# chrischoy/DeepGlobalRegistration

Hardware: AMD Instinct MI355X
Metric: pair registrations/sec (FCGF x2 + 1-NN + 6-D inlier net + gate + weighted Procrustes + SE(3) refinement) (higher is better)
Workload: dtype f32 results via 2 x f16 split operands (3 f16 MFMA products per MAC, f32 accumulate); k = 1 convs, kNN re-evaluation and registration in exact f32, SVD in f64

## Files before the change

deepglobalregistration_amd/_lib.py:

```python
import ctypes as C
import os
import threading

import torch

_HERE = os.path.dirname(os.path.abspath(__file__))
LIB_PATH = os.environ.get('DGR_HIP_LIB') or os.path.join(_HERE, 'lib', 'libdgr_hip.so')

DGR_OK, DGR_EINVAL, DGR_EHIP, DGR_ENOMEM, DGR_ESVD, DGR_EINTERNAL = 0, -1, -2, -3, -4, -5
STATUS_OK, STATUS_LOW_CONFIDENCE, STATUS_SVD_FAILED, STATUS_SAFEGUARD = 0, 1, 2, 3
STATUS_FLAG_ICP_SKIPPED, STATUS_MASK = 0x100, 0xff

c_i32p, c_i64p, c_f32p, c_f64p = (C.POINTER(C.c_int32), C.POINTER(C.c_int64),
                                  C.POINTER(C.c_float), C.POINTER(C.c_double))
vp = C.c_void_p


class WeightDesc(C.Structure):
    _fields_ = [('name', C.c_char_p), ('data', vp), ('numel', C.c_int64)]


class Params(C.Structure):
    _fields_ = [('clip_weight_thresh', C.c_float), ('voxel_size', C.c_float),
                ('inlier_feature_type', C.c_int), ('max_iter', C.c_int),
# ... 12 lines not shown
    'dgr_ctx_create': (C.c_int, [C.c_int, C.POINTER(vp)]),
    'dgr_ctx_destroy': (None, [vp]),
    'dgr_ctx_workspace_bytes': (C.c_int64, [vp]),
    'dgr_ctx_create_partition_stream': (C.c_int, [vp, C.c_int, C.c_int, C.POINTER(vp)]),
    'dgr_voxelize': (C.c_int, [vp, vp, C.c_int, C.c_int64, C.c_double, C.c_int32, vp, vp, vp, c_i64p, vp]),
    'dgr_net_create': (C.c_int, [vp, C.c_int, C.c_int, C.c_int, C.c_int, C.c_int,
                                 C.POINTER(WeightDesc), C.c_int, C.POINTER(vp)]),
    'dgr_net_create_device': (C.c_int, [vp, C.c_int, C.c_int, C.c_int, C.c_int, C.c_int,
                                        C.POINTER(WeightDesc), C.c_int, C.POINTER(vp)]),
    'dgr_net_destroy': (None, [vp]),
    'dgr_net_param_bytes': (C.c_int64, [vp]),
    'dgr_net_share': (C.c_int, [vp, vp, C.POINTER(vp)]),
    'dgr_net_sharers': (C.c_int, [vp]),
    'dgr_resunet_forward': (C.c_int, [vp, vp, vp, vp, C.c_int64, vp, vp]),
    'dgr_net_get_intermediate': (C.c_int, [vp, vp, C.c_char_p, vp, C.c_int64, c_i64p, c_i64p]),
    'dgr_net_layer_stats': (C.c_int, [vp, vp, C.c_int, c_i64p]),
    'dgr_net_num_layers': (C.c_int, [vp]),
    'dgr_net_rerun_layer': (C.c_int, [vp, vp, C.c_int, C.c_int, c_f32p, c_f32p]),
    'dgr_maps_create': (C.c_int, [vp, vp, C.c_int64, C.c_int, C.c_int, C.POINTER(vp), vp]),
    'dgr_maps_destroy': (None, [vp]),
    'dgr_maps_get_coords': (C.c_int, [vp, C.c_int, vp, C.c_int64, c_i64p]),
    'dgr_maps_get_kernel_map': (C.c_int, [vp, C.c_int, C.c_int, vp, C.c_int64, vp, vp, C.c_int64,
                                          c_i64p, c_i64p]),
    'dgr_knn1_l2': (C.c_int, [vp, vp, C.c_int64, vp, C.c_int64, C.c_int, C.c_int, vp, vp, vp]),
    'dgr_knn1_l2_batch': (C.c_int, [vp, vp, c_i64p, vp, c_i64p, C.c_int, C.c_int, C.c_int, vp, vp, vp]),
    'dgr_knn_l2': (C.c_int, [vp, vp, C.c_int64, vp, C.c_int64, C.c_int, C.c_int, C.c_int, vp, vp, vp]),
    'dgr_knn_l2_batch': (C.c_int, [vp, vp, c_i64p, vp, c_i64p, C.c_int, C.c_int, C.c_int, C.c_int, vp, vp,
                                   vp]),
    'dgr_inlier_inputs': (C.c_int, [vp, vp, vp, C.c_int64, vp, vp, C.c_int64, vp, C.c_int, vp, vp, vp]),
    'dgr_sigmoid_clip_sum': (C.c_int, [vp, vp, C.c_int64, C.c_float, vp, c_f64p, vp]),
    'dgr_gather_rows3': (C.c_int, [vp, vp, vp, C.c_int64, vp, vp]),
    'dgr_weighted_procrustes': (C.c_int, [vp, vp, vp, vp, C.c_int64, C.c_float, c_f32p, c_f32p, vp]),
    'dgr_se3_refine': (C.c_int, [vp, vp, vp, vp, C.c_int64, C.c_float, C.c_int, C.c_int, C.c_double,
                                 c_f32p, c_f32p, c_i32p, c_f32p, c_i32p, vp]),
    'dgr_register_batch': (C.c_int, [vp, vp, vp, vp, vp, c_i64p, vp, vp, c_i64p, C.c_int,
                                     C.POINTER(Params), vp, vp, c_f32p, c_i32p, c_f32p, vp]),
    'dgr_register_pairs': (C.c_int, [vp, vp, vp, vp, vp, c_i64p, C.c_int, C.c_int, c_i32p, C.c_int,
                                     C.POINTER(Params), vp, vp, c_f32p, c_i32p, c_f32p, vp]),
    'dgr_register_batch_f64': (C.c_int, [vp, c_f64p, C.c_int64, c_i64p]),
    'dgr_register_batch_output': (C.c_int, [vp, C.c_int, vp, C.c_int64, c_i64p, vp]),
    'dgr_ctx_set_profiling': (C.c_int, [vp, C.c_int]),
    'dgr_icp_point_to_point': (C.c_int, [vp, vp, C.c_int64, vp, C.c_int64, C.c_double, c_f64p, C.c_int, C.c_double,
                                          C.c_double, c_f64p, c_f64p, vp]),
    'dgr_ransac_correspondence': (C.c_int, [vp, vp, vp, C.c_int64, C.c_double, C.c_int64, C.c_uint32, c_f64p, c_f64p, vp]),
    'dgr_ctx_stage_times': (C.c_int, [vp, c_f32p]),
    'dgr_ctx_stage_times_v2': (C.c_int, [vp, c_f32p, C.c_int, C.POINTER(C.c_int)]),
# ... 109 lines not shown
```

deepglobalregistration_amd/csrc/coordmap.hip:

```cpp
#include <algorithm>

#include "dgr_internal.h"
#include "hash.h"

constexpr int SCAN_THREADS = 256;
constexpr int SCAN_ITEMS = 8;
constexpr int SCAN_BLOCK = SCAN_THREADS * SCAN_ITEMS;

__device__ __forceinline__ int block_exclusive_scan_256(int v, int *lds , int *total) {
  const int lane = threadIdx.x & 63, wave = threadIdx.x >> 6;
  int x = v;
#pragma unroll
  for (int d = 1; d < 64; d <<= 1) {
    int y = __shfl_up(x, d, 64);
    if (lane >= d) x += y;
  }
  if (lane == 63) lds[wave] = x;
  __syncthreads();
  int base = 0, tot = 0;
#pragma unroll
  for (int w = 0; w < SCAN_THREADS / 64; ++w) {
    int s = lds[w];
    if (w < wave) base += s;
    tot += s;
// ... 288 lines not shown
}

__global__ void half_keys_kernel(const int32_t *__restrict__ coords7, const int32_t *n_dev,
                                 int32_t *__restrict__ keys4) {
  int64_t r = (int64_t)blockIdx.x * blockDim.x + threadIdx.x;
  if (r >= *n_dev) return;
#pragma unroll
  for (int d = 0; d < 4; ++d) keys4[r * 4 + d] = coords7[r * 7 + d];
}

__global__ void bucket_count_kernel(const int32_t *__restrict__ keys4, const int32_t *n_dev,
                                    const int32_t *__restrict__ table, uint32_t mask,
                                    const int32_t *__restrict__ bkeys, int32_t *__restrict__ row_bucket,
                                    int32_t *counts) {
  int64_t r = (int64_t)blockIdx.x * blockDim.x + threadIdx.x;
  if (r >= *n_dev) return;
  int32_t q[4] = {keys4[r * 4], keys4[r * 4 + 1], keys4[r * 4 + 2], keys4[r * 4 + 3]};
  const int b = dgr_lookup<4>(table, mask, bkeys, q);
  row_bucket[r] = b;
  atomicAdd(&counts[b], 1);
}

__global__ void bucket_members_kernel(const int32_t *__restrict__ row_bucket, const int32_t *n_dev,
                                      const int32_t *__restrict__ start, int32_t *cursor, int32_t *__restrict__ members) {
  int64_t r = (int64_t)blockIdx.x * blockDim.x + threadIdx.x;
  if (r >= *n_dev) return;
  const int b = row_bucket[r];
  members[start[b] + atomicAdd(&cursor[b], 1)] = (int32_t)r;
}

__global__ void bucket_fill_kernel(const int32_t *__restrict__ row_bucket, const int32_t *n_dev,
                                   const int32_t *__restrict__ start, int32_t *cursor,
                                   const int32_t *__restrict__ members,
                                   const int32_t *__restrict__ coords7, int4 *__restrict__ second,
                                   int32_t *__restrict__ coords_new, int32_t *__restrict__ canon, int32_t *__restrict__ inv) {
  int64_t r = (int64_t)blockIdx.x * blockDim.x + threadIdx.x;
  if (r >= *n_dev) return;
  const int b = row_bucket[r];
  const int32_t *c = coords7 + r * 7;
  int p;
  if (members) {
    int rank = 0;
    for (int e = start[b], end = start[b + 1]; e < end; ++e) rank += members[e] < (int32_t)r;
    p = start[b] + rank;
  } else {
    p = start[b] + atomicAdd(&cursor[b], 1);
  }
  if (coords_new) {
#pragma unroll
    for (int d = 0; d < 7; ++d) coords_new[(int64_t)p * 7 + d] = c[d];
    canon[p] = (int32_t)r;
    inv[r] = p;
    second[p] = make_int4(c[4], c[5], c[6], p);
  } else {
    second[p] = make_int4(c[4], c[5], c[6], (int32_t)r);
  }
}

struct RenumberJobs {
  const int32_t *inv[4];
  int32_t *table[4];
  uint32_t cap[4];
};
__global__ void renumber_table_kernel(RenumberJobs j) {
  const int l = blockIdx.y;
  const uint32_t s = blockIdx.x * blockDim.x + threadIdx.x;
  if (s >= j.cap[l]) return;
  const int v = j.table[l][s];
  if (v >= 0) j.table[l][s] = j.inv[l][v];
}
// ... 52 lines not shown
  }
  DGR_LAUNCH_CHECK();
  {
    const int32_t *ins[4];
    int32_t *outs[4], *tots[4];
    int64_t ns[4];
    for (int l = 0; l < levels; ++l) { ins[l] = counts[l]; outs[l] = hb[l].start; tots[l] = nullptr; ns[l] = cm[l].n_cap + 1; }
    DGR_CHECK(dgr_exclusive_scan_multi(arena, levels, ins, outs, ns, tots, stream));
  }
  RenumberJobs rj = {};
  int nrj = 0;
  int64_t max_cap = 0;
  for (int l = 0; l < levels; ++l) {
    const int64_t n = cm[l].n_cap;
    int32_t *coords_new = nullptr, *canon = nullptr, *inv = nullptr;
    if (l >= renumber_from) {
      DGR_ALLOC(coords_new, arena, int32_t, n * 7);
      DGR_ALLOC(canon, arena, int32_t, n);
      DGR_ALLOC(inv, arena, int32_t, n);
      rj.inv[nrj] = inv; rj.table[nrj] = cm[l].table; rj.cap[nrj] = cm[l].table_mask + 1;
      max_cap = std::max<int64_t>(max_cap, rj.cap[nrj]);
      ++nrj;
    }
    const int32_t *members = nullptr;
    if (coords_new) {
      bucket_members_kernel<<<grid_for(n), 256, 0, stream>>>(row_bucket[l], cm[l].n_dev, hb[l].start, cursor[l], rank[l]);
      members = rank[l];
    }
    bucket_fill_kernel<<<grid_for(n), 256, 0, stream>>>(row_bucket[l], cm[l].n_dev, hb[l].start, cursor[l], members,
                                                        cm[l].coords, hb[l].second, coords_new, canon, inv);
    if (coords_new) { cm[l].coords = coords_new; cm[l].canon = canon; }
    hb[l].built = true;
  }
  if (nrj) renumber_table_kernel<<<dim3((unsigned)grid_for(max_cap), nrj), 256, 0, stream>>>(rj);
  DGR_LAUNCH_CHECK();
  return DGR_OK;
}

int dgr_build_coord_maps(DgrArena &arena, const int32_t *coords, int64_t N, DgrMapSet *ms,
                         hipStream_t stream) {
  if (ms->nc == 4) return build_coord_maps_t<4>(arena, coords, N, ms, stream);
  if (ms->nc == 7) return build_coord_maps_t<7>(arena, coords, N, ms, stream);
  dgr_set_error("unsupported dimension D=%d (3 and 6 are on the DGR path)", ms->D);
  return DGR_EINVAL;
}

template <typename T>
__global__ void voxel_keys(const T *__restrict__ xyz, int64_t M, T inv_unused, T voxel, int32_t batch,
                           int32_t *__restrict__ keys) {
  int64_t r = (int64_t)blockIdx.x * blockDim.x + threadIdx.x;
  if (r >= M) return;
  keys[r * 4] = batch;
#pragma unroll
// ... 53 lines not shown
```

deepglobalregistration_amd/csrc/dgr_internal.h:

```cpp
#pragma once
#include <hip/hip_runtime.h>
#include <stdint.h>
#include <stdio.h>
#include <stdlib.h>
#include <string>
#include <vector>

#include "../../include/dgr_hip.h"

void dgr_set_error(const char *fmt, ...);

#define DGR_HIP_CHECK(expr)                                                                  \
  do {                                                                                       \
    hipError_t _e = (expr);                                                                  \
    if (_e != hipSuccess) {                                                                  \
      dgr_set_error("%s:%d: %s failed: %s", __FILE__, __LINE__, #expr, hipGetErrorString(_e)); \
      return DGR_EHIP;                                                                       \
    }                                                                                        \
  } while (0)

#define DGR_CHECK(expr)          \
  do {                           \
    int _r = (expr);             \
    if (_r != DGR_OK) return _r; \
// ... 59 lines not shown
};

struct DgrHalfBuckets {
  int32_t *bkeys = nullptr;
  int32_t *table = nullptr;
  uint32_t mask = 0;
  int32_t *start = nullptr;
  int4 *second = nullptr;
  bool built = false;
};

struct DgrKernelMap {
  int K = 0;
  int32_t *rule_ptr = nullptr;
  int32_t *tile_ptr = nullptr;
  int4 *tile_desc = nullptr;
  int64_t tile_cap = 0;
  int32_t *pair_in = nullptr;
  int32_t *pair_out = nullptr;
  int32_t *out_ptr = nullptr, *out_pos = nullptr;
  uint16_t *pair_k = nullptr;
  int32_t *in_ptr = nullptr, *in_pos = nullptr;
  int64_t pair_cap = 0;
  bool built = false;
};

constexpr int DGR_OS_ROWS = 64;
struct DgrNbrTable {
  int32_t *nbr = nullptr;
  int64_t n_pad = 0;
  int K = 27;
  bool built = false;
  int32_t *perm = nullptr, *cls_count = nullptr;
  int64_t cls_cap = 0;
};

struct DgrMapSet {
  int D = 3, nc = 4, conv1_ks = 3;
  bool use_nbr = false;
  DgrNbrTable nsame[4];
  DgrNbrTable ndown[3];
  DgrNbrTable nup[3];
  DgrCoordMap cm[4];
  DgrHalfBuckets hb[4];
  DgrKernelMap same[4];
  DgrKernelMap conv1;
// ... 181 lines not shown
```

deepglobalregistration_amd/csrc/kmap.hip:

```cpp
#include <string.h>

#include <algorithm>

#include "dgr_internal.h"
#include "hash.h"

constexpr int KM_THREADS = 256;

template <int D>
__device__ __forceinline__ void offset_of(int k, int ks, int ts, int32_t *delta) {
  const int half = ks >> 1;
#pragma unroll
  for (int d = 0; d < D; ++d) {
    delta[d] = ((k % ks) - half) * ts;
    k /= ks;
  }
}

template <int D>
__device__ __forceinline__ int probe(const int32_t *__restrict__ out_coords, int64_t o,
                                     const int32_t *delta, const int32_t *__restrict__ in_coords,
                                     const int32_t *__restrict__ in_table, uint32_t in_mask) {
  constexpr int NC = D + 1;
  int32_t q[NC];
// ... 79 lines not shown
#pragma unroll
    for (int i = 0; i < KW; ++i) {
      J.wpre[m][r * KW + i] = (unsigned short)c;
      c += __popc(w[i]);
    }
  }
  J.cnt[m][r] = c;
}
__device__ __forceinline__ int mask_rank_pre(const uint32_t *__restrict__ m, const unsigned short *__restrict__ pre, int k) {
  return pre[k >> 5] + __popc(m[k >> 5] & ((1u << (k & 31)) - 1u));
}


__device__ __forceinline__ unsigned long long hit_pack(int k, int64_t o, int64_t in) {
  return ((unsigned long long)k << 54) | ((unsigned long long)o << 27) | (unsigned long long)in;
}
constexpr int KM_REGION = 512;
constexpr int KM_JOBS6 = 8;
struct HitList {
  unsigned long long *recs;
  int32_t *wave_count;
  int region;
};
__device__ __forceinline__ void hit_begin(volatile int *cur) {
  if ((threadIdx.x & 63) == 0) cur[threadIdx.x >> 6] = 0;
}
__device__ __forceinline__ int64_t hit_slots(int n, const HitList &h, volatile int *cur, int wave_id) {
  const unsigned long long act = __ballot(1), two = __ballot(n == 2);
  const int lane = threadIdx.x & 63, w = threadIdx.x >> 6;
  const unsigned long long below = (1ull << lane) - 1ull;
  int base = 0;
  if (lane == __ffsll((long long)act) - 1) {
    base = cur[w];
    const int need = __popcll(act) + __popcll(two);
    if (base >= 0 && base + need <= h.region) {
      cur[w] = base + need;
    } else {
      cur[w] = -1;
      base = -1;
    }
  }
  base = __builtin_amdgcn_readfirstlane(base);
  if (base < 0) return -1;
  return (int64_t)wave_id * h.region + base + __popcll(act & below) + __popcll(two & below);
}
__device__ __forceinline__ void hit_end(const HitList &h, volatile int *cur, int wave_id) {
  if ((threadIdx.x & 63) == 0) h.wave_count[wave_id] = cur[threadIdx.x >> 6];
}

struct PrunedArgs {
  const int32_t *out_coords, *n_out_dev;
  const int4 *out_order;
  int64_t n_cap;
  DgrHalfBuckets hb;
  int ts_in, symmetric;
};
template <class Emit>
__device__ __forceinline__ void pruned_search6(const PrunedArgs &a, int64_t t, Emit &&emit) {
  const int NJ = a.symmetric ? 14 : 27;
  const int ts_in = a.ts_in;
  const int ja = (int)(t / a.n_cap);
  const int64_t p = t - (int64_t)ja * a.n_cap;
  int b = -1;
  int64_t o = 0;
  int c4 = 0, c5 = 0, c6 = 0;
  if (ja < NJ && p < *a.n_out_dev) {
    const int4 me = a.out_order[p];
    o = me.w; c4 = me.x; c5 = me.y; c6 = me.z;
    const int32_t *co = a.out_coords + o * 7;
    int32_t q[4];
    q[0] = co[0];
    q[1] = co[1] + ((ja % 3) - 1) * ts_in;
    q[2] = co[2] + (((ja / 3) % 3) - 1) * ts_in;
    q[3] = co[3] + ((ja / 9) - 1) * ts_in;
    b = dgr_lookup<4>(a.hb.table, a.hb.mask, a.hb.bkeys, q);
  }
  const int beg = b >= 0 ? a.hb.start[b] : 0, end = b >= 0 ? a.hb.start[b + 1] : 0;
  for (int p0 = beg; p0 < end; p0 += 4) {
    int4 e[4];
#pragma unroll
    for (int u = 0; u < 4; ++u) e[u] = a.hb.second[min(p0 + u, end - 1)];
#pragma unroll
    for (int u = 0; u < 4; ++u) {
      if (p0 + u >= end) break;
      const int d4 = e[u].x - c4, d5 = e[u].y - c5, d6 = e[u].z - c6;
      if (abs(d4) <= ts_in && abs(d5) <= ts_in && abs(d6) <= ts_in) {
        const int k = ja + 27 * ((d4 / ts_in + 1) + 3 * (d5 / ts_in + 1) + 9 * (d6 / ts_in + 1));
        if (a.symmetric && ja == 13 && k > 364) continue;
        emit(k, o, e[u].w);
      }
    }
  }
}

struct Bits6Jobs {
  PrunedArgs pa[KM_JOBS6];
  uint32_t *mask_out[KM_JOBS6], *mask_in[KM_JOBS6];
  HitList hl[KM_JOBS6];
  int blocks[KM_JOBS6];
};
__global__ void __launch_bounds__(KM_THREADS)
    kmap_bits_pruned6(Bits6Jobs J, int KW) {
  __shared__ int hit_cur[KM_THREADS / 64];
  const int jm = blockIdx.y;
  if ((int)blockIdx.x >= J.blocks[jm]) return;
  const PrunedArgs a = J.pa[jm];
  uint32_t *const mask_out = J.mask_out[jm], *const mask_in = J.mask_in[jm];
  const HitList hl = J.hl[jm];
  hit_begin(hit_cur);
  const int wid = (int)(blockIdx.x * (KM_THREADS / 64) + (threadIdx.x >> 6));
  pruned_search6(a, (int64_t)blockIdx.x * KM_THREADS + threadIdx.x, [&](int k, int64_t o, int in) {
    atomicOr(&mask_out[o * KW + (k >> 5)], 1u << (k & 31));
    const int km = 728 - k;
    if (a.symmetric) {
      if (km != k) atomicOr(&mask_out[(int64_t)in * KW + (km >> 5)], 1u << (km & 31));
    } else if (mask_in) {
      atomicOr(&mask_in[(int64_t)in * KW + (k >> 5)], 1u << (k & 31));
    }
    const int n = (a.symmetric && km != k) ? 2 : 1;
    const int64_t s = hit_slots(n, hl, hit_cur, wid);
    if (s >= 0) {
      hl.recs[s] = hit_pack(k, o, in);
      if (n == 2) hl.recs[s + 1] = hit_pack(km, in, o);
    }
  });
  hit_end(hl, hit_cur, wid);
}

constexpr int KM_KMAX = 736;
struct Colmask6Jobs {
  const uint32_t *mask_out[KM_JOBS6];
  const int32_t *n_out_dev[KM_JOBS6];
  int RB[KM_JOBS6];
  int4 *cell[KM_JOBS6];
  int32_t *counts[KM_JOBS6], *row_cnt[KM_JOBS6];
  unsigned short *wpre[KM_JOBS6];
};
__global__ void __launch_bounds__(KM_THREADS)
    kmap_colmask(Colmask6Jobs J, int K, int KW) {
  __shared__ unsigned long long bal[KM_THREADS / 64][KM_KMAX];
  const int jm = blockIdx.y;
  const int RB = J.RB[jm];
  if ((int)blockIdx.x >= RB) return;
  const uint32_t *__restrict__ mask_out = J.mask_out[jm];
  const int32_t *n_out_dev = J.n_out_dev[jm];
  int4 *__restrict__ cell = J.cell[jm];
  int32_t *__restrict__ counts = J.counts[jm], *__restrict__ row_cnt = J.row_cnt[jm];
// ... 48 lines not shown
  int64_t pair_cap;
  int32_t *overflow;
  const uint32_t *mask_in;
  const int32_t *in_ptr;
  int32_t *in_pos;
  const unsigned short *wpre_out, *wpre_in;
};
__device__ __forceinline__ void place_pair(const PlaceArgs &p, int k, int64_t o, int64_t in) {
  const int64_t slot = (int64_t)p.out_ptr[o] + mask_rank_pre(p.mask_out + o * p.KW, p.wpre_out + o * p.KW, k);
  const int64_t g = o >> 6;
  const int4 c = p.cell[g * p.K + k];
  const unsigned long long cm = ((unsigned long long)(uint32_t)c.y << 32) | (uint32_t)c.x;
  const int64_t pos = (int64_t)p.base[(int64_t)k * p.RB + (g >> 2)] + c.z + __popcll(cm & ((1ull << (o & 63)) - 1ull));
  if (pos < p.pair_cap && slot < p.pair_cap) {
    p.pair_in[pos] = (int32_t)in;
    if (p.pair_out) p.pair_out[pos] = (int32_t)o;
    if (p.pair_k) p.pair_k[pos] = (uint16_t)k;
    p.out_pos[slot] = (int32_t)pos;
    if (p.mask_in) p.in_pos[p.in_ptr[in] + mask_rank_pre(p.mask_in + in * p.KW, p.wpre_in + in * p.KW, k)] = (int32_t)pos;
  } else {
    *p.overflow = 2;
  }
}

struct Place6Jobs {
  HitList h[KM_JOBS6];
  PlaceArgs p[KM_JOBS6];
  PrunedArgs replay[KM_JOBS6];
  int n_waves[KM_JOBS6], blocks[KM_JOBS6];
};
__global__ void __launch_bounds__(KM_THREADS)
    kmap_place_hits(Place6Jobs J) {
  const int jm = blockIdx.y;
  const int nblk = J.blocks[jm];
  if ((int)blockIdx.x >= nblk) return;
  const HitList h = J.h[jm];
  const PlaceArgs p = J.p[jm];
  const PrunedArgs replay = J.replay[jm];
  const int n_waves = J.n_waves[jm];
  const int lane = threadIdx.x & 63;
  for (int r = blockIdx.x * (KM_THREADS / 64) + (threadIdx.x >> 6); r < n_waves; r += nblk * (KM_THREADS / 64)) {
    const int n = h.wave_count[r];
    if (n < 0) {
      pruned_search6(replay, (int64_t)r * 64 + lane, [&](int k, int64_t o, int in) {
        place_pair(p, k, o, in);
        if (replay.symmetric && 728 - k != k) place_pair(p, 728 - k, in, o);
      });
      continue;
    }
    for (int e = lane; e < n; e += 64) {
      const unsigned long long rec = h.recs[(int64_t)r * h.region + e];
      place_pair(p, (int)(rec >> 54), (int64_t)((rec >> 27) & 0x7ffffffull), (int64_t)(rec & 0x7ffffffull));
    }
  }
}

constexpr int KM_KGROUP = 8;
__global__ void __launch_bounds__(KM_THREADS)
    kmap_fill(const int32_t *n_out_dev, int RB, int K, int64_t n_cap, const int32_t *__restrict__ hits,
              const int32_t *__restrict__ block_counts, const int32_t *__restrict__ block_base,
              int32_t *__restrict__ pair_in, int32_t *__restrict__ pair_out, int64_t pair_cap,
              int32_t *overflow, int KW, const uint32_t *__restrict__ mask_out,
              const int32_t *__restrict__ out_ptr, int32_t *__restrict__ out_pos,
              const uint32_t *__restrict__ mask_in, const int32_t *__restrict__ in_ptr,
              int32_t *__restrict__ in_pos, uint16_t *__restrict__ pair_k) {
  __shared__ int wave_cnt[2][KM_THREADS / 64];
  const int rb = blockIdx.x;
  const int n_out = *n_out_dev;
  if (rb * KM_THREADS >= n_out) return;
  const int lane = threadIdx.x & 63, wave = threadIdx.x >> 6;
  const int64_t o = (int64_t)rb * KM_THREADS + threadIdx.x;
  int parity = 0;
  for (int kk = 0; kk < KM_KGROUP; ++kk) {
    const int k = blockIdx.y * KM_KGROUP + kk;
    if (k >= K) break;
// ... 140 lines not shown
    int32_t *outs[3] = {km->out_ptr, base, km->in_ptr}, *tots[3] = {nullptr, total, nullptr};
    const int64_t ns[3] = {n_cap + 1, (int64_t)K * RB, n_in_cap + 1};
    DGR_CHECK(dgr_exclusive_scan_multi(arena, need_in_csr ? 3 : 2, ins, outs, ns, tots, stream));
  }
  FinalizeJobs fj = {};
  finalize_job(fj, 0, base, total, K, RB, km);
  kmap_finalize<<<1, 1024, 0, stream>>>(fj);
  tile_desc_kernel<<<dim3((unsigned)dgr_ceil_div(km->tile_cap, 256), 1), 256, 0, stream>>>(fj);
  kmap_fill<<<dim3(RB, (K + KM_KGROUP - 1) / KM_KGROUP), KM_THREADS, 0, stream>>>(
      out.n_dev, RB, K, n_cap, hits, counts, base, km->pair_in, km->pair_out, km->pair_cap, overflow, KW, mask_out,
      km->out_ptr, km->out_pos, mask_in, km->in_ptr, km->in_pos, km->pair_k);
  DGR_LAUNCH_CHECK();
  arena.rewind(mk);
  km->built = true;
  return DGR_OK;
}

struct Kmap6Job {
  const DgrCoordMap *in, *out;
  const DgrHalfBuckets *hb;
  const DgrHalfBuckets *hb_out;
  bool need_in_csr, want_pair_out, want_pair_k;
  DgrKernelMap *km;
};
static int build_kernel_maps6(DgrArena &arena, const Kmap6Job *jobs, int nj, int max_pairs_per_row, int32_t *overflow,
                              hipStream_t stream) {
  constexpr int K = 729, KW = (K + 31) / 32;
  DGR_REQUIRE(nj >= 1 && nj <= KM_MAXJOBS, "6-D kernel maps: %d jobs", nj);
  struct Tr {
    int RB, symmetric;
    int64_t n_cap, n_in_cap, hit_waves;
    int32_t *counts, *base, *total, *cnt_out, *cnt_in;
    uint32_t *mask_out, *mask_in;
    int4 *cell;
    HitList hl;
    unsigned short *wpre_out, *wpre_in;
  } t[KM_MAXJOBS];
  for (int m = 0; m < nj; ++m) {
    const Kmap6Job &J = jobs[m];
    t[m].n_cap = J.out->n_cap; t[m].n_in_cap = J.in->n_cap;
    DGR_REQUIRE(t[m].n_cap < (1ll << 27) && t[m].n_in_cap < (1ll << 27), "6-D kernel maps: more than 2^27 rows");
    DGR_CHECK(alloc_kernel_map(arena, K, t[m].n_cap, t[m].n_in_cap, max_pairs_per_row, J.need_in_csr, J.want_pair_out,
                               J.want_pair_k, J.km));
  }
  DgrArena::Mark mk = arena.mark();
  {
    size_t words = 0;
    for (int m = 0; m < nj; ++m)
      words += (size_t)(t[m].n_cap + 1) * KW + (jobs[m].need_in_csr ? (size_t)(t[m].n_in_cap + 1) * KW : 0) + (size_t)(t[m].n_cap + 1);
    uint32_t *pool;
    DGR_ALLOC(pool, arena, uint32_t, words);
    DGR_HIP_CHECK(hipMemsetAsync(pool, 0, words * sizeof(uint32_t), stream));
    for (int m = 0; m < nj; ++m) {
      t[m].mask_out = pool; pool += (size_t)(t[m].n_cap + 1) * KW;
      t[m].mask_in = nullptr;
      if (jobs[m].need_in_csr) { t[m].mask_in = pool; pool += (size_t)(t[m].n_in_cap + 1) * KW; }
      t[m].cnt_out = reinterpret_cast<int32_t *>(pool); pool += (size_t)(t[m].n_cap + 1);
    }
  }
  for (int m = 0; m < nj; ++m) {
    const Kmap6Job &J = jobs[m];
    Tr &r = t[m];
    r.RB = (int)dgr_ceil_div(r.n_cap, KM_THREADS);
    r.symmetric = (J.in->coords == J.out->coords && !J.need_in_csr) ? 1 : 0;
    DGR_REQUIRE(J.hb && J.hb->built && J.hb_out && J.hb_out->built, "6-D kernel map: first-half buckets missing");
    DGR_ALLOC(r.counts, arena, int32_t, (int64_t)K * r.RB);
// ... 10 lines not shown
    DGR_ALLOC(r.hl.wave_count, arena, int32_t, r.hit_waves);
    DGR_ALLOC(r.wpre_out, arena, unsigned short, (r.n_cap + 1) * KW);
    r.wpre_in = nullptr;
    if (J.need_in_csr) DGR_ALLOC(r.wpre_in, arena, unsigned short, (r.n_in_cap + 1) * KW);
  }
  static_assert(KM_JOBS6 >= KM_MAXJOBS, "multi-job launch tables");
  {
    Bits6Jobs bj = {};
    Colmask6Jobs cj = {};
    int max_sb = 0, max_rb = 0;
    for (int m = 0; m < nj; ++m) {
      const Kmap6Job &J = jobs[m];
      Tr &r = t[m];
      bj.pa[m] = PrunedArgs{J.out->coords, J.out->n_dev, J.hb_out->second, r.n_cap, *J.hb, J.in->ts, r.symmetric};
      bj.mask_out[m] = r.mask_out; bj.mask_in[m] = r.mask_in; bj.hl[m] = r.hl;
      bj.blocks[m] = (int)(r.hit_waves / (KM_THREADS / 64));
      max_sb = std::max(max_sb, bj.blocks[m]);
      cj.mask_out[m] = r.mask_out; cj.n_out_dev[m] = J.out->n_dev; cj.RB[m] = r.RB; cj.cell[m] = r.cell;
      cj.counts[m] = r.counts; cj.row_cnt[m] = r.cnt_out; cj.wpre[m] = r.wpre_out;
      max_rb = std::max(max_rb, r.RB);
    }
    kmap_bits_pruned6<<<dim3((unsigned)max_sb, (unsigned)nj), KM_THREADS, 0, stream>>>(bj, KW);
    kmap_colmask<<<dim3((unsigned)max_rb, (unsigned)nj), KM_THREADS, 0, stream>>>(cj, K, KW);
    {
      MaskCountJobs mj = {};
      int nm = 0;
      long long max_rows = 0;
      for (int m = 0; m < nj; ++m)
        if (jobs[m].need_in_csr) {
          mj.mask[nm] = t[m].mask_in; mj.n_dev[nm] = jobs[m].in->n_dev; mj.n_cap[nm] = t[m].n_in_cap + 1;
          mj.cnt[nm] = t[m].cnt_in; mj.wpre[nm] = t[m].wpre_in;
          max_rows = std::max(max_rows, mj.n_cap[nm]);
          ++nm;
        }
      static_assert(KM_MC_JOBS >= KM_MAXJOBS, "mask-count job table");
      if (nm) mask_count_multi<KW><<<dim3((unsigned)dgr_ceil_div(max_rows, 256), (unsigned)nm), 256, 0, stream>>>(mj);
    }
  }
  DGR_LAUNCH_CHECK();
  {
    const int32_t *ins[DGR_SCAN_MAX];
    int32_t *outs[DGR_SCAN_MAX], *tots[DGR_SCAN_MAX];
    int64_t ns[DGR_SCAN_MAX];
    int c = 0;
    for (int m = 0; m < nj; ++m) {
      ins[c] = t[m].cnt_out; outs[c] = jobs[m].km->out_ptr; tots[c] = nullptr; ns[c++] = t[m].n_cap + 1;
// ... 229 lines not shown
      for (int l = 0; l < 3; ++l) {
        cj.coords[l] = ms->cm[l].coords; cj.n_dev[l] = ms->cm[l].n_dev; cj.ts[l] = ms->cm[l].ts;
        cj.nb[l] = (int)dgr_ceil_div(ms->cm[l].n_cap, KM_THREADS);
        DGR_ALLOC(cj.blk_cnt[l], arena, int32_t, (int64_t)cj.nb[l] * 8);
        cj.perm[l] = ms->nup[l].perm; cj.cls_count[l] = ms->nup[l].cls_count; cj.cls_cap[l] = ms->nup[l].cls_cap;
        max_nb = std::max(max_nb, cj.nb[l]);
      }
      cls_count_kernel<<<dim3((unsigned)max_nb, 3), KM_THREADS, 0, stream>>>(cj);
      cls_fill_kernel<<<dim3((unsigned)max_nb, 3), KM_THREADS, 0, stream>>>(cj);
      DGR_LAUNCH_CHECK();
    }
    if (lean) {
      if (conv1_ks != 3 && !skip_conv1_map)
        DGR_CHECK(build_kernel_map3(arena, ms->cm[0], ms->cm[0], conv1_ks, 1024, false, false, true, &ms->conv1, ms->overflow,
                                    stream));
      return DGR_OK;
    }
  }
  const int cap_row = (D == 3) ? 1024 : 160;
  if (D == 6) {
    DGR_REQUIRE(conv1_ks == 3, "6-D kernel maps support kernel size 3 only (got %d)", conv1_ks);
    DGR_CHECK(dgr_build_half_buckets(arena, ms->cm, ms->hb, 4, 1, stream));
    Kmap6Job jobs[7];
    for (int l = 0; l < 4; ++l) jobs[l] = {&ms->cm[l], &ms->cm[l], &ms->hb[l], &ms->hb[l], false, !lean, !lean || l == 0, &ms->same[l]};
    for (int l = 0; l < 3; ++l) jobs[4 + l] = {&ms->cm[l], &ms->cm[l + 1], &ms->hb[l], &ms->hb[l + 1], true, true, !lean, &ms->down[l]};
    DGR_CHECK(build_kernel_maps6(arena, jobs, 7, cap_row, ms->overflow, stream));
    ms->conv1 = ms->same[0];
    return DGR_OK;
  }
  auto build = [&](const DgrCoordMap &in, const DgrCoordMap &out, int ks, bool rev, bool want_k, DgrKernelMap *km) -> int {
    const bool want_out = !lean || rev, want_pk = !lean || want_k;
    return build_kernel_map3(arena, in, out, ks, cap_row, rev, want_out, want_pk, km, ms->overflow, stream);
  };
  for (int l = 0; l < 4; ++l) DGR_CHECK(build(ms->cm[l], ms->cm[l], 3, false, l == 0, &ms->same[l]));
  if (conv1_ks == 3)
    ms->conv1 = ms->same[0];
  else if (!skip_conv1_map)
    DGR_CHECK(build(ms->cm[0], ms->cm[0], conv1_ks, false, true, &ms->conv1));
  for (int l = 0; l < 3; ++l) DGR_CHECK(build(ms->cm[l], ms->cm[l + 1], 3, true, false, &ms->down[l]));
  return DGR_OK;
}

struct dgr_maps {
  dgr_ctx *ctx;
  DgrArena arena;
  DgrMapSet ms;
  int32_t *coords_copy = nullptr;
  hipStream_t stream;
// ... 124 lines not shown
        if (!c.canon) return DGR_OK;
        int32_t n = 0;
        DGR_HIP_CHECK(hipMemcpy(&n, c.n_dev, sizeof(int32_t), hipMemcpyDeviceToHost));
        v.resize(n);
        DGR_HIP_CHECK(hipMemcpy(v.data(), c.canon, (size_t)n * sizeof(int32_t), hipMemcpyDeviceToHost));
        return DGR_OK;
      };
      std::vector<int32_t> ci, co, rp(km->K + 1);
      DGR_CHECK(fetch(cin, ci));
      DGR_CHECK(fetch(cout, co));
      DGR_HIP_CHECK(hipMemcpy(rp.data(), km->rule_ptr, rp.size() * sizeof(int32_t), hipMemcpyDeviceToHost));
      std::vector<std::pair<int32_t, int32_t>> tmp;
      for (int k = 0; k < km->K; ++k) {
        tmp.clear();
        for (int32_t q = rp[k]; q < rp[k + 1]; ++q)
          tmp.push_back({cout.canon ? co[pair_out[q]] : pair_out[q], cin.canon ? ci[pair_in[q]] : pair_in[q]});
        std::sort(tmp.begin(), tmp.end());
        for (size_t u = 0; u < tmp.size(); ++u) { pair_out[rp[k] + u] = tmp[u].first; pair_in[rp[k] + u] = tmp[u].second; }
      }
    }
  }
  return DGR_OK;
}
```

deepglobalregistration_amd/ops.py:

```python
import ctypes as C

import numpy as np
import torch

from . import _lib
from ._lib import check, get_ctx, ptr, stream_ptr, vp

F32_EPS = float(np.finfo(np.float32).eps)


def _dev(t):
    if not (torch.is_tensor(t) and t.is_cuda):
        raise ValueError('expected a CUDA(ROCm) tensor')
    return t.device


def _as(t, dtype, device):
    if not torch.is_tensor(t):
        t = torch.as_tensor(np.asarray(t))
    return t.to(device=device, dtype=dtype).contiguous()


def voxelize(xyz, voxel_size, batch_index=0, device='cuda'):
    lib = _lib.load()
# ... 155 lines not shown
        except Exception:
            pass

    def coords(self, ts):
        lib = _lib.load()
        n = C.c_int64(0)
        check(lib.dgr_maps_get_coords(self.handle, ts, None, 0, C.byref(n)))
        out = np.empty((n.value, self.D + 1), np.int32)
        check(lib.dgr_maps_get_coords(self.handle, ts, out.ctypes.data, out.size, C.byref(n)))
        return out

    def kernel_map(self, kind, ts):
        lib = _lib.load()
        kid = {'same': 0, 'conv1': 1, 'down': 2, 'nbr_same': 3, 'nbr_down': 4, 'nbr_up': 5}[kind]
        K, P = C.c_int64(0), C.c_int64(0)
        check(lib.dgr_maps_get_kernel_map(self.handle, kid, ts, None, 0, None, None, 0, C.byref(K), C.byref(P)))
        rule = np.empty(K.value + 1, np.int32)
        pin = np.empty(P.value, np.int32)
        pout = np.empty(P.value, np.int32)
        check(lib.dgr_maps_get_kernel_map(self.handle, kid, ts, rule.ctypes.data, rule.size, pin.ctypes.data,
                                          pout.ctypes.data, pin.size, C.byref(K), C.byref(P)))
        k = np.repeat(np.arange(K.value), np.diff(rule))
        return k.astype(np.int64), pin.astype(np.int64), pout.astype(np.int64)


def knn1(F0, F1, squared=False, return_distance=False):
    lib = _lib.load()
    dev = _dev(F0)
    F0 = _as(F0, torch.float32, dev)
    F1 = _as(F1, torch.float32, dev)
    if F0.dim() != 2 or F1.dim() != 2 or F0.shape[1] != F1.shape[1]:
        raise ValueError('F0 [N0,C] and F1 [N1,C] must share the feature width')
    N0, N1 = F0.shape[0], F1.shape[0]
    idx = torch.empty(N0, dtype=torch.int64, device=dev)
    dist = torch.empty(N0, dtype=torch.float32, device=dev) if return_distance else None
    check(lib.dgr_knn1_l2(get_ctx(dev), ptr(F0), N0, ptr(F1), N1, F0.shape[1], int(squared), ptr(idx),
                          ptr(dist), stream_ptr(dev.index)))
    return (idx, dist) if return_distance else idx


def knn1_batch(F0, F1, off0, off1, squared=False, return_distance=False):
    lib = _lib.load()
    dev = _dev(F0)
    F0 = _as(F0, torch.float32, dev)
    F1 = _as(F1, torch.float32, dev)
    if F0.dim() != 2 or F1.dim() != 2 or F0.shape[1] != F1.shape[1]:
# ... 598 lines not shown
```

include/dgr_hip.h:

```cpp
#ifndef DGR_HIP_H
#define DGR_HIP_H

#include <stdint.h>

#ifdef __cplusplus
extern "C" {
#endif

typedef struct dgr_ctx dgr_ctx;
typedef struct dgr_net dgr_net;
typedef struct dgr_maps dgr_maps;
typedef void *dgr_stream;

enum {
  DGR_OK = 0,
  DGR_EINVAL = -1,
  DGR_EHIP = -2,
  DGR_ENOMEM = -3,
  DGR_ESVD = -4,
  DGR_EINTERNAL = -5
};

enum { DGR_STATUS_OK = 0, DGR_STATUS_LOW_CONFIDENCE = 1, DGR_STATUS_SVD_FAILED = 2,
       DGR_STATUS_SAFEGUARD = 3 ,
// ... 24 lines not shown
int dgr_net_create_device(dgr_ctx *ctx, int D, int in_channels, int out_channels, int conv1_kernel_size,
                          int normalize_feature, const dgr_weight_desc *weights, int n_weights,
                          dgr_net **out);
void dgr_net_destroy(dgr_net *net);
int64_t dgr_net_param_bytes(const dgr_net *net);
int dgr_net_share(dgr_ctx *ctx, const dgr_net *src, dgr_net **out);
int dgr_net_sharers(const dgr_net *net);

int dgr_resunet_forward(dgr_ctx *ctx, dgr_net *net, const int32_t *coords, const float *feats,
                        int64_t N, float *out, dgr_stream stream);
int dgr_net_get_intermediate(dgr_ctx *ctx, dgr_net *net, const char *name, float *host_out,
                             int64_t capacity, int64_t *rows, int64_t *cols);
int dgr_net_layer_stats(dgr_ctx *ctx, dgr_net *net, int layer, int64_t stats[8]);
int dgr_net_num_layers(const dgr_net *net);
int dgr_net_rerun_layer(dgr_ctx *ctx, dgr_net *net, int layer, int reps, float *gemm_ms, float *reduce_ms);

int dgr_maps_create(dgr_ctx *ctx, const int32_t *coords, int64_t N, int D, int conv1_kernel_size,
                    dgr_maps **out, dgr_stream stream);
void dgr_maps_destroy(dgr_maps *maps);
int dgr_maps_get_coords(dgr_maps *maps, int ts, int32_t *host_out, int64_t capacity, int64_t *n);
int dgr_maps_get_kernel_map(dgr_maps *maps, int kind, int ts, int32_t *rule_ptr, int64_t rule_cap,
                            int32_t *pair_in, int32_t *pair_out, int64_t pair_cap, int64_t *K,
                            int64_t *P);

int dgr_knn1_l2(dgr_ctx *ctx, const float *F0, int64_t N0, const float *F1, int64_t N1, int C,
                int squared, int64_t *idx_out, float *dist_out, dgr_stream stream);

int dgr_knn1_l2_batch(dgr_ctx *ctx, const float *F0, const int64_t *off0, const float *F1,
                      const int64_t *off1, int npairs, int C, int squared, int64_t *idx_out,
                      float *dist_out, dgr_stream stream);

#define DGR_KNN_MAX_K 32
int dgr_knn_l2(dgr_ctx *ctx, const float *F0, int64_t N0, const float *F1, int64_t N1, int C, int k,
               int squared, int64_t *idx_out, float *dist_out, dgr_stream stream);

int dgr_knn_l2_batch(dgr_ctx *ctx, const float *F0, const int64_t *off0, const float *F1,
                     const int64_t *off1, int npairs, int C, int k, int squared, int64_t *idx_out,
                     float *dist_out, dgr_stream stream);

int dgr_inlier_inputs(dgr_ctx *ctx, const int32_t *coords0, const float *xyz0, int64_t N0,
                      const int32_t *coords1, const float *xyz1, int64_t N1, const int64_t *idx1,
                      int feature_type, int32_t *coords6_out, float *feats_out, dgr_stream stream);

int dgr_sigmoid_clip_sum(dgr_ctx *ctx, const float *logit, int64_t N, float clip, float *weights_out,
                         double *wsum, dgr_stream stream);

// ... 101 lines not shown
```

Baseline: 392.1.

## Sort half-bucket members by x and binary-search the 6-D kernel-map candidate range

Half-bucket members are now always sorted by their x coordinate, then by row, using int2 (row, x) member records. This lets the pruned 6-D kernel-map search binary-search the start of the x window and stop early once past the upper bound, instead of scanning whole buckets. The hit list now stores only one record per hit, and the symmetric mirror pair is produced at placement time, which halves hit-list traffic and replays. It also adds debug APIs for CSR export and hit statistics, plus a stats kernel that runs only in non-lean builds. The sorting pass now always runs, which adds a members kernel launch even when coordinates are not reordered.

```diff
diff --git a/deepglobalregistration_amd/_lib.py b/deepglobalregistration_amd/_lib.py
--- a/deepglobalregistration_amd/_lib.py
+++ b/deepglobalregistration_amd/_lib.py
@@ -58,6 +58,9 @@
     'dgr_maps_get_coords': (C.c_int, [vp, C.c_int, vp, C.c_int64, c_i64p]),
     'dgr_maps_get_kernel_map': (C.c_int, [vp, C.c_int, C.c_int, vp, C.c_int64, vp, vp, C.c_int64,
                                           c_i64p, c_i64p]),
+    'dgr_maps_get_kernel_map_csr': (C.c_int, [vp, C.c_int, C.c_int, C.c_int, vp, C.c_int64, vp, vp, C.c_int64, c_i64p,
+                                              c_i64p]),
+    'dgr_maps_get_hit_stats': (C.c_int, [vp, C.c_int, C.c_int, c_i64p, c_i64p]),
     'dgr_knn1_l2': (C.c_int, [vp, vp, C.c_int64, vp, C.c_int64, C.c_int, C.c_int, vp, vp, vp]),
     'dgr_knn1_l2_batch': (C.c_int, [vp, vp, c_i64p, vp, c_i64p, C.c_int, C.c_int, C.c_int, vp, vp, vp]),
     'dgr_knn_l2': (C.c_int, [vp, vp, C.c_int64, vp, C.c_int64, C.c_int, C.c_int, C.c_int, vp, vp, vp]),
diff --git a/deepglobalregistration_amd/csrc/coordmap.hip b/deepglobalregistration_amd/csrc/coordmap.hip
--- a/deepglobalregistration_amd/csrc/coordmap.hip
+++ b/deepglobalregistration_amd/csrc/coordmap.hip
@@ -334,30 +334,29 @@
 }
 
 __global__ void bucket_members_kernel(const int32_t *__restrict__ row_bucket, const int32_t *n_dev,
-                                      const int32_t *__restrict__ start, int32_t *cursor, int32_t *__restrict__ members) {
+                                      const int32_t *__restrict__ start, int32_t *cursor,
+                                      const int32_t *__restrict__ coords7, int2 *__restrict__ members) {
   int64_t r = (int64_t)blockIdx.x * blockDim.x + threadIdx.x;
   if (r >= *n_dev) return;
   const int b = row_bucket[r];
-  members[start[b] + atomicAdd(&cursor[b], 1)] = (int32_t)r;
+  members[start[b] + atomicAdd(&cursor[b], 1)] = make_int2((int32_t)r, coords7[r * 7 + 4]);
 }
 
 __global__ void bucket_fill_kernel(const int32_t *__restrict__ row_bucket, const int32_t *n_dev,
-                                   const int32_t *__restrict__ start, int32_t *cursor,
-                                   const int32_t *__restrict__ members,
+                                   const int32_t *__restrict__ start, const int2 *__restrict__ members,
                                    const int32_t *__restrict__ coords7, int4 *__restrict__ second,
                                    int32_t *__restrict__ coords_new, int32_t *__restrict__ canon, int32_t *__restrict__ inv) {
   int64_t r = (int64_t)blockIdx.x * blockDim.x + threadIdx.x;
   if (r >= *n_dev) return;
   const int b = row_bucket[r];
   const int32_t *c = coords7 + r * 7;
-  int p;
-  if (members) {
-    int rank = 0;
-    for (int e = start[b], end = start[b + 1]; e < end; ++e) rank += members[e] < (int32_t)r;
-    p = start[b] + rank;
-  } else {
-    p = start[b] + atomicAdd(&cursor[b], 1);
-  }
+  const int x1 = c[4];
+  int rank = 0;
+  for (int e = start[b], end = start[b + 1]; e < end; ++e) {
+    const int2 m = members[e];
+    rank += (m.y < x1) || (m.y == x1 && m.x < (int32_t)r);
+  }
+  const int p = start[b] + rank;
   if (coords_new) {
 #pragma unroll
     for (int d = 0; d < 7; ++d) coords_new[(int64_t)p * 7 + d] = c[d];
@@ -456,13 +455,10 @@
       max_cap = std::max<int64_t>(max_cap, rj.cap[nrj]);
       ++nrj;
     }
-    const int32_t *members = nullptr;
-    if (coords_new) {
-      bucket_members_kernel<<<grid_for(n), 256, 0, stream>>>(row_bucket[l], cm[l].n_dev, hb[l].start, cursor[l], rank[l]);
-      members = rank[l];
-    }
-    bucket_fill_kernel<<<grid_for(n), 256, 0, stream>>>(row_bucket[l], cm[l].n_dev, hb[l].start, cursor[l], members,
-                                                        cm[l].coords, hb[l].second, coords_new, canon, inv);
+    int2 *members = reinterpret_cast<int2 *>(keys[l]);
+    bucket_members_kernel<<<grid_for(n), 256, 0, stream>>>(row_bucket[l], cm[l].n_dev, hb[l].start, cursor[l], cm[l].coords, members);
+    bucket_fill_kernel<<<grid_for(n), 256, 0, stream>>>(row_bucket[l], cm[l].n_dev, hb[l].start, members, cm[l].coords,
+                                                        hb[l].second, coords_new, canon, inv);
     if (coords_new) { cm[l].coords = coords_new; cm[l].canon = canon; }
     hb[l].built = true;
   }
diff --git a/deepglobalregistration_amd/csrc/dgr_internal.h b/deepglobalregistration_amd/csrc/dgr_internal.h
--- a/deepglobalregistration_amd/csrc/dgr_internal.h
+++ b/deepglobalregistration_amd/csrc/dgr_internal.h
@@ -105,6 +105,7 @@
   uint16_t *pair_k = nullptr;
   int32_t *in_ptr = nullptr, *in_pos = nullptr;
   int64_t pair_cap = 0;
+  unsigned long long *hit_stats = nullptr;
   bool built = false;
 };
 
diff --git a/deepglobalregistration_amd/csrc/kmap.hip b/deepglobalregistration_amd/csrc/kmap.hip
--- a/deepglobalregistration_amd/csrc/kmap.hip
+++ b/deepglobalregistration_amd/csrc/kmap.hip
@@ -125,17 +125,26 @@
   int32_t *wave_count;
   int region;
 };
+__global__ void kmap_hit_stats(HitList h, int n_waves, unsigned long long *stats) {
+  unsigned long long recs = 0, replays = 0;
+  for (int w = blockIdx.x * blockDim.x + threadIdx.x; w < n_waves; w += gridDim.x * blockDim.x) {
+    const int n = h.wave_count[w];
+    if (n < 0) ++replays; else recs += (unsigned long long)n;
+  }
+  if (recs) atomicAdd(&stats[0], recs);
+  if (replays) atomicAdd(&stats[1], replays);
+}
 __device__ __forceinline__ void hit_begin(volatile int *cur) {
   if ((threadIdx.x & 63) == 0) cur[threadIdx.x >> 6] = 0;
 }
-__device__ __forceinline__ int64_t hit_slots(int n, const HitList &h, volatile int *cur, int wave_id) {
-  const unsigned long long act = __ballot(1), two = __ballot(n == 2);
+__device__ __forceinline__ int64_t hit_slot(const HitList &h, volatile int *cur, int wave_id) {
+  const unsigned long long act = __ballot(1);
   const int lane = threadIdx.x & 63, w = threadIdx.x >> 6;
   const unsigned long long below = (1ull << lane) - 1ull;
   int base = 0;
   if (lane == __ffsll((long long)act) - 1) {
     base = cur[w];
-    const int need = __popcll(act) + __popcll(two);
+    const int need = __popcll(act);
     if (base >= 0 && base + need <= h.region) {
       cur[w] = base + need;
     } else {
@@ -145,7 +154,7 @@
   }
   base = __builtin_amdgcn_readfirstlane(base);
   if (base < 0) return -1;
-  return (int64_t)wave_id * h.region + base + __popcll(act & below) + __popcll(two & below);
+  return (int64_t)wave_id * h.region + base + __popcll(act & below);
 }
 __device__ __forceinline__ void hit_end(const HitList &h, volatile int *cur, int wave_id) {
   if ((threadIdx.x & 63) == 0) h.wave_count[wave_id] = cur[threadIdx.x >> 6];
@@ -178,7 +187,18 @@
     q[3] = co[3] + ((ja / 9) - 1) * ts_in;
     b = dgr_lookup<4>(a.hb.table, a.hb.mask, a.hb.bkeys, q);
   }
-  const int beg = b >= 0 ? a.hb.start[b] : 0, end = b >= 0 ? a.hb.start[b + 1] : 0;
+  int beg = b >= 0 ? a.hb.start[b] : 0;
+  const int end = b >= 0 ? a.hb.start[b + 1] : 0;
+  if (end - beg > 4) {
+    const int x_lo = c4 - ts_in;
+    int lo = beg, hi = end;
+    while (lo < hi) {
+      const int mid = (lo + hi) >> 1;
+      if (a.hb.second[mid].x < x_lo) lo = mid + 1; else hi = mid;
+    }
+    beg = lo;
+  }
+  const int x_hi = c4 + ts_in;
   for (int p0 = beg; p0 < end; p0 += 4) {
     int4 e[4];
 #pragma unroll
@@ -193,6 +213,7 @@
         emit(k, o, e[u].w);
       }
     }
+    if (e[3].x > x_hi) break;
   }
 }
 
@@ -220,12 +241,8 @@
     } else if (mask_in) {
       atomicOr(&mask_in[(int64_t)in * KW + (k >> 5)], 1u << (k & 31));
     }
-    const int n = (a.symmetric && km != k) ? 2 : 1;
-    const int64_t s = hit_slots(n, hl, hit_cur, wid);
-    if (s >= 0) {
-      hl.recs[s] = hit_pack(k, o, in);
-      if (n == 2) hl.recs[s + 1] = hit_pack(km, in, o);
-    }
+    const int64_t s = hit_slot(hl, hit_cur, wid);
+    if (s >= 0) hl.recs[s] = hit_pack(k, o, in);
   });
   hit_end(hl, hit_cur, wid);
 }
@@ -320,6 +337,10 @@
     *p.overflow = 2;
   }
 }
+__device__ __forceinline__ void place_hit_symmetric(const PlaceArgs &p, int k, int64_t o, int64_t in) {
+  place_pair(p, k, o, in);
+  if (728 - k != k) place_pair(p, 728 - k, in, o);
+}
 
 struct Place6Jobs {
   HitList h[KM_JOBS6];
@@ -341,14 +362,15 @@
     const int n = h.wave_count[r];
     if (n < 0) {
       pruned_search6(replay, (int64_t)r * 64 + lane, [&](int k, int64_t o, int in) {
-        place_pair(p, k, o, in);
-        if (replay.symmetric && 728 - k != k) place_pair(p, 728 - k, in, o);
+        if (replay.symmetric) place_hit_symmetric(p, k, o, in); else place_pair(p, k, o, in);
       });
       continue;
     }
     for (int e = lane; e < n; e += 64) {
       const unsigned long long rec = h.recs[(int64_t)r * h.region + e];
-      place_pair(p, (int)(rec >> 54), (int64_t)((rec >> 27) & 0x7ffffffull), (int64_t)(rec & 0x7ffffffull));
+      const int k = (int)(rec >> 54);
+      const int64_t o = (int64_t)((rec >> 27) & 0x7ffffffull), in = (int64_t)(rec & 0x7ffffffull);
+      if (replay.symmetric) place_hit_symmetric(p, k, o, in); else place_pair(p, k, o, in);
     }
   }
 }
@@ -535,6 +557,7 @@
   const DgrHalfBuckets *hb_out;
   bool need_in_csr, want_pair_out, want_pair_k;
   DgrKernelMap *km;
+  bool want_hit_stats = false;
 };
 static int build_kernel_maps6(DgrArena &arena, const Kmap6Job *jobs, int nj, int max_pairs_per_row, int32_t *overflow,
                               hipStream_t stream) {
@@ -555,6 +578,11 @@
     DGR_REQUIRE(t[m].n_cap < (1ll << 27) && t[m].n_in_cap < (1ll << 27), "6-D kernel maps: more than 2^27 rows");
     DGR_CHECK(alloc_kernel_map(arena, K, t[m].n_cap, t[m].n_in_cap, max_pairs_per_row, J.need_in_csr, J.want_pair_out,
                                J.want_pair_k, J.km));
+    J.km->hit_stats = nullptr;
+    if (J.want_hit_stats) {
+      DGR_ALLOC(J.km->hit_stats, arena, unsigned long long, 2);
+      DGR_HIP_CHECK(hipMemsetAsync(J.km->hit_stats, 0, 2 * sizeof(unsigned long long), stream));
+    }
   }
   DgrArena::Mark mk = arena.mark();
   {
@@ -611,6 +639,10 @@
     }
     kmap_bits_pruned6<<<dim3((unsigned)max_sb, (unsigned)nj), KM_THREADS, 0, stream>>>(bj, KW);
     kmap_colmask<<<dim3((unsigned)max_rb, (unsigned)nj), KM_THREADS, 0, stream>>>(cj, K, KW);
+    for (int m = 0; m < nj; ++m)
+      if (jobs[m].km->hit_stats)
+        kmap_hit_stats<<<(unsigned)std::min<int64_t>(dgr_ceil_div(t[m].hit_waves, 256), 1024), 256, 0, stream>>>(
+            t[m].hl, (int)t[m].hit_waves, jobs[m].km->hit_stats);
     {
       MaskCountJobs mj = {};
       int nm = 0;
@@ -886,8 +918,8 @@
     DGR_REQUIRE(conv1_ks == 3, "6-D kernel maps support kernel size 3 only (got %d)", conv1_ks);
     DGR_CHECK(dgr_build_half_buckets(arena, ms->cm, ms->hb, 4, 1, stream));
     Kmap6Job jobs[7];
-    for (int l = 0; l < 4; ++l) jobs[l] = {&ms->cm[l], &ms->cm[l], &ms->hb[l], &ms->hb[l], false, !lean, !lean || l == 0, &ms->same[l]};
-    for (int l = 0; l < 3; ++l) jobs[4 + l] = {&ms->cm[l], &ms->cm[l + 1], &ms->hb[l], &ms->hb[l + 1], true, true, !lean, &ms->down[l]};
+    for (int l = 0; l < 4; ++l) jobs[l] = {&ms->cm[l], &ms->cm[l], &ms->hb[l], &ms->hb[l], false, !lean, !lean || l == 0, &ms->same[l], !lean};
+    for (int l = 0; l < 3; ++l) jobs[4 + l] = {&ms->cm[l], &ms->cm[l + 1], &ms->hb[l], &ms->hb[l + 1], true, true, !lean, &ms->down[l], !lean};
     DGR_CHECK(build_kernel_maps6(arena, jobs, 7, cap_row, ms->overflow, stream));
     ms->conv1 = ms->same[0];
     return DGR_OK;
@@ -1058,3 +1090,55 @@
   }
   return DGR_OK;
 }
+
+static int kernel_map_of(dgr_maps *m, int kind, int ts, const DgrKernelMap **km, int *l_out) {
+  const int l = level_of(ts);
+  DGR_REQUIRE(l >= 0, "tensor stride %d not in {1,2,4,8}", ts);
+  *km = nullptr;
+  if (kind == 0) *km = &m->ms.same[l];
+  else if (kind == 1) *km = &m->ms.conv1;
+  else if (kind == 2 && l < 3) *km = &m->ms.down[l];
+  DGR_REQUIRE(*km && (*km)->built, "no such kernel map (kind %d, ts %d)", kind, ts);
+  *l_out = l;
+  return DGR_OK;
+}
+
+extern "C" int dgr_maps_get_kernel_map_csr(dgr_maps *m, int kind, int ts, int side, int32_t *ptr, int64_t ptr_cap, int32_t *pos,
+                                           int32_t *pair_row, int64_t pair_cap, int64_t *n_rows, int64_t *P) {
+  DGR_REQUIRE(m && n_rows && P && (side == 0 || side == 1), "dgr_maps_get_kernel_map_csr: bad argument");
+  const DgrKernelMap *km;
+  int l;
+  DGR_CHECK(kernel_map_of(m, kind, ts, &km, &l));
+  const DgrCoordMap &rows = side == 0 ? m->ms.cm[kind == 2 ? l + 1 : l] : m->ms.cm[l];
+  const int32_t *dptr = side == 0 ? km->out_ptr : km->in_ptr, *dpos = side == 0 ? km->out_pos : km->in_pos;
+  const int32_t *drow = side == 0 ? km->pair_out : km->pair_in;
+  DGR_REQUIRE(dptr && dpos && drow, "kernel map (kind %d, ts %d) has no %s-major CSR", kind, ts, side ? "input" : "output");
+  int32_t n32 = 0, total = 0;
+  DGR_HIP_CHECK(hipMemcpy(&n32, rows.n_dev, sizeof(int32_t), hipMemcpyDeviceToHost));
+  DGR_HIP_CHECK(hipMemcpy(&total, km->rule_ptr + km->K, sizeof(int32_t), hipMemcpyDeviceToHost));
+  *n_rows = n32;
+  *P = total;
+  if (ptr) {
+    DGR_REQUIRE(ptr_cap >= (int64_t)n32 + 1, "ptr buffer too small");
+    DGR_HIP_CHECK(hipMemcpy(ptr, dptr, ((size_t)n32 + 1) * sizeof(int32_t), hipMemcpyDeviceToHost));
+  }
+  if (pos && pair_row) {
+    DGR_REQUIRE(pair_cap >= total, "pair buffers too small");
+    DGR_HIP_CHECK(hipMemcpy(pos, dpos, (size_t)total * sizeof(int32_t), hipMemcpyDeviceToHost));
+    DGR_HIP_CHECK(hipMemcpy(pair_row, drow, (size_t)total * sizeof(int32_t), hipMemcpyDeviceToHost));
+  }
+  return DGR_OK;
+}
+
+extern "C" int dgr_maps_get_hit_stats(dgr_maps *m, int kind, int ts, int64_t *records, int64_t *replayed_waves) {
+  DGR_REQUIRE(m && records && replayed_waves, "NULL argument");
+  const DgrKernelMap *km;
+  int l;
+  DGR_CHECK(kernel_map_of(m, kind, ts, &km, &l));
+  DGR_REQUIRE(km->hit_stats, "kernel map (kind %d, ts %d) was not built through a hit list", kind, ts);
+  unsigned long long host[2];
+  DGR_HIP_CHECK(hipMemcpy(host, km->hit_stats, sizeof(host), hipMemcpyDeviceToHost));
+  *records = (int64_t)host[0];
+  *replayed_waves = (int64_t)host[1];
+  return DGR_OK;
+}
diff --git a/deepglobalregistration_amd/ops.py b/deepglobalregistration_amd/ops.py
--- a/deepglobalregistration_amd/ops.py
+++ b/deepglobalregistration_amd/ops.py
@@ -201,6 +201,29 @@
                                           pout.ctypes.data, pin.size, C.byref(K), C.byref(P)))
         k = np.repeat(np.arange(K.value), np.diff(rule))
         return k.astype(np.int64), pin.astype(np.int64), pout.astype(np.int64)
+
+    _KINDS = {'same': 0, 'conv1': 1, 'down': 2}
+
+    def kernel_map_csr(self, kind, ts, side='out'):
+        lib = _lib.load()
+        kid, sid = self._KINDS[kind], {'out': 0, 'in': 1}[side]
+        n, P, K, P2 = C.c_int64(0), C.c_int64(0), C.c_int64(0), C.c_int64(0)
+        check(lib.dgr_maps_get_kernel_map_csr(self.handle, kid, ts, sid, None, 0, None, None, 0, C.byref(n), C.byref(P)))
+        ptr_ = np.empty(n.value + 1, np.int32)
+        pos = np.empty(P.value, np.int32)
+        row = np.empty(P.value, np.int32)
+        check(lib.dgr_maps_get_kernel_map_csr(self.handle, kid, ts, sid, ptr_.ctypes.data, ptr_.size, pos.ctypes.data,
+                                              row.ctypes.data, pos.size, C.byref(n), C.byref(P)))
+        check(lib.dgr_maps_get_kernel_map(self.handle, kid, ts, None, 0, None, None, 0, C.byref(K), C.byref(P2)))
+        rule = np.empty(K.value + 1, np.int32)
+        check(lib.dgr_maps_get_kernel_map(self.handle, kid, ts, rule.ctypes.data, rule.size, None, None, 0, C.byref(K),
+                                          C.byref(P2)))
+        return ptr_, pos, row, rule
+
+    def hit_stats(self, kind, ts):
+        rec, rep = C.c_int64(0), C.c_int64(0)
+        check(_lib.load().dgr_maps_get_hit_stats(self.handle, self._KINDS[kind], ts, C.byref(rec), C.byref(rep)))
+        return rec.value, rep.value
 
 
 def knn1(F0, F1, squared=False, return_distance=False):
diff --git a/include/dgr_hip.h b/include/dgr_hip.h
--- a/include/dgr_hip.h
+++ b/include/dgr_hip.h
@@ -70,6 +70,9 @@
 int dgr_maps_get_kernel_map(dgr_maps *maps, int kind, int ts, int32_t *rule_ptr, int64_t rule_cap,
                             int32_t *pair_in, int32_t *pair_out, int64_t pair_cap, int64_t *K,
                             int64_t *P);
+int dgr_maps_get_kernel_map_csr(dgr_maps *maps, int kind, int ts, int side, int32_t *ptr, int64_t ptr_cap, int32_t *pos,
+                                int32_t *pair_row, int64_t pair_cap, int64_t *n_rows, int64_t *P);
+int dgr_maps_get_hit_stats(dgr_maps *maps, int kind, int ts, int64_t *records, int64_t *replayed_waves);
 
 int dgr_knn1_l2(dgr_ctx *ctx, const float *F0, int64_t N0, const float *F1, int64_t N1, int C,
                 int squared, int64_t *idx_out, float *dist_out, dgr_stream stream);
```

New measurement: 396.9, median of 6. 1.01x the previous value.
